# rogermm14/eonerf_code

Measured on AMD Instinct MI355X. Metric: train rays/sec on JAX_068 (4096 rays x 128 samples), higher is better.
Workload: dtype bf16

## Files before the change

eonerf_code_amd/csrc/eonerf_ctx.h:

```cpp
#pragma once
#include <hip/hip_runtime.h>
#include <string.h>
#include <algorithm>
#include <vector>
#include <unordered_map>

#include "../../include/eonerf_hip.h"
#include "eonerf_kernels.h"
#include "eonerf_pack.h"
#include "eonerf_rays.h"
#include "eonerf_carve.h"
#include "eonerf_wgrad_plan.h"

#define HIP_TRY(x) do { hipError_t e_ = (x); if (e_ != hipSuccess) return (int)e_; } while (0)

struct DevStream {
    uint8_t* data = nullptr; size_t bytes = 0;
    ChunkDesc* chunks = nullptr; int n_chunks = 0;
    PackEntry *e16 = nullptr, *e32 = nullptr, *e16lo = nullptr; int n16 = 0, n32 = 0, n16lo = 0;
};

constexpr int RANGE_WORD = 16;
constexpr int RANGE_STICKY_WORD = 17;
constexpr int DIGEST_WORD = 32;

struct eonerf_ctx {
    eonerf_config cfg;
    int n_samples = 128;
    int prec;
    bool bf16;
    int n_cu;
    int enc_pair = 1;
    int pipe_xcd = 0;
    int stagger = 0;
    int wgrad_riders = 1;
    ParamLayout pl;
    DevStream fwd_full, fwd_dens, bwd_full, bwd_dens, bwd_rgb, bwd_full_ig, pipe_wt, bwd_full_heads, bwd_rgb_heads, bwd_dens_heads, ig_tail_wt;
    bool pipe = false;
    int n_pipes = 0;
    float* loss_scratch = nullptr;
    float* fold = nullptr;
    bool pipe_fallback = true;
    bool need_repack = false;
    std::unordered_map<const void*, bool> ws_pipe;
    int pipe_fault_stage = -1;
    bool deterministic = false;
    unsigned long long* pipe_stamps = nullptr;
    uint64_t noise_seed = 0x5eed5eedULL; uint32_t noise_call = 0;
    struct Presample { bool valid = false; const void* ws = nullptr; const float* rays = nullptr; const int64_t* img_idx = nullptr;
                       const float* zsteps = nullptr; const int* count_out = nullptr; int n_rays = 0, flags = 0, n_samples = 0; bool pipe = false; uint32_t call = 0; } pre;
    hipEvent_t exch_event = nullptr; int exch_cus = 0; bool exch_recorded = false;
    const void* pre_consumed_ws = nullptr;
    bool full_ig_dirty = false;
    int* enc_colmap = nullptr;
    int* dev_status = nullptr;
    const uint32_t* occ_bits = nullptr; int occ_r = 0;
    bool weights_set = false;
    bool dens_dirty = false;
    bool dens_used = false;
    int prof_cap = 0;
    std::vector<hipEvent_t> prof_ev[EONERF_PROF_KERNELS][2];
    int prof_n[EONERF_PROF_KERNELS] = {};
};

inline CarveCfg carve_cfg(const eonerf_ctx* ctx) {
    CarveCfg c;
    c.bf16 = ctx->bf16; c.pipe = ctx->pipe; c.deterministic = ctx->deterministic; c.pipe_partials = ctx->deterministic;
    c.n_pipes = ctx->n_pipes; c.n_samples = ctx->n_samples;
    c.enc_part_wgs = (ctx->enc_pair && ctx->pipe && !ctx->deterministic) ? ctx->n_cu : 0;
    return c;
}
inline RenderWs carve_render(const eonerf_ctx* ctx, void* base, int n_rays, int flags) { return carve_render(carve_cfg(ctx), base, n_rays, flags); }

struct ProfScope {
    eonerf_ctx* c; int k; hipStream_t st; bool on;
    ProfScope(eonerf_ctx* ctx, int kernel, hipStream_t s) : c(ctx), k(kernel), st(s), on(kernel >= 0 && ctx->prof_cap > 0 && ctx->prof_n[kernel] < ctx->prof_cap) {
        if (on) (void)hipEventRecord(c->prof_ev[k][0][c->prof_n[k]], st);
    }
    ~ProfScope() { if (on) { (void)hipEventRecord(c->prof_ev[k][1][c->prof_n[k]], st); c->prof_n[k]++; } }
};

inline bool slabs_addressable(const eonerf_ctx* ctx, size_t p_cap) { return slab_blocks_addressable(ctx->bf16, p_cap); }
inline void drop_presample(eonerf_ctx* ctx, const void* ws) { if (ctx->pre.valid && ctx->pre.ws == ws) ctx->pre.valid = false; }
inline bool rays_in_range(const eonerf_ctx* ctx, int n_rays) { return n_rays <= (1 << 24) / (ctx->n_samples > 128 ? ctx->n_samples / 128 : 1); }
inline int chain_grid(const eonerf_ctx* ctx, int p_cap) { return std::min(ctx->n_cu, p_cap / (ctx->bf16 ? PBf16::TILE : PF32::TILE)); }

inline void note_train_forward(eonerf_ctx* ctx, const void* ws) {
    if (ctx->ws_pipe.size() > 1024) ctx->ws_pipe.clear();
    ctx->ws_pipe[ws] = ctx->pipe;
}
struct PipeModeGuard {
    eonerf_ctx* c; bool keep; const void* ws_; bool spend;
    PipeModeGuard(eonerf_ctx* ctx, const void* ws, bool spend_record = true) : c(ctx), keep(ctx->pipe), ws_(ws), spend(spend_record) {
        auto it = c->ws_pipe.find(ws);
        if (it != c->ws_pipe.end()) c->pipe = it->second;
    }
    ~PipeModeGuard() { c->pipe = keep; if (spend) c->ws_pipe.erase(ws_); }
};

inline AmbientW ambient_w(const eonerf_ctx* ctx, const float* flat) {
    const ParamLayout& pl = ctx->pl;
    return AmbientW{flat + pl.t[pl.am1_w].offset, flat + pl.t[pl.am1_b].offset, flat + pl.t[pl.am2_w].offset, flat + pl.t[pl.am2_b].offset};
}

inline int pipe_spare_cus(const eonerf_ctx* ctx) {
    const int spare = ctx->n_cu - ctx->n_pipes * PIPE_STAGES;
    return (ctx->pipe && !ctx->deterministic && spare >= 2) ? std::min(spare, 8) : 0;
}

inline MlpBwdArgs mlp_bwd_args(const eonerf_ctx* ctx, const PassBuffers& b, int p_cap, const DevStream& bs) {
    MlpBwdArgs m;
    memset(&m, 0, sizeof(m));
    m.stagger = ctx->stagger;
    m.n_pts = b.n_pts; m.p_pad = p_cap;
    m.stream = bs.data; m.chunks = bs.chunks; m.n_chunks = bs.n_chunks;
    m.sigma = b.sigma; m.albedo = b.albedo; m.ts = b.ts; m.tb = b.tb;
    m.g_sigma = b.g_sigma; m.g_albedo = b.g_albedo; m.g_ts = b.g_ts; m.g_tb = b.g_tb;
    m.masks = b.masks; m.grd = b.grd; m.g_emb = b.g_emb;
    m.px = b.px; m.py = b.py; m.pz = b.pz; m.g_pos = b.g_pos;
    return m;
}

int eo_pack(const eonerf_ctx* ctx, const std::vector<const DevStream*>& streams, const float* flat, hipStream_t st);
int eo_ensure_density_streams(eonerf_ctx* ctx, const float* flat, hipStream_t st);
int eo_sample_rays(eonerf_ctx* ctx, const float* rays, const float* zsteps, const float* u, int perturb, int n_rays, const uint32_t* bits, int r,
                   int64_t* ray_indices, float* t_starts, float* t_ends, float* pts_per_ray, int* n_dev, void* ws, size_t ws_bytes, void* stream);
int eo_run_mlp_fwd(eonerf_ctx* ctx, const PassBuffers& b, const float* flat, int p_cap, bool full, int mode, hipStream_t st, int prof_id = -1, bool render_train = false);
int eo_run_weight_gradients(eonerf_ctx* ctx, const float* flat, float* d_flat, const PassBuffers* full, const PassBuffers* dens, int p_cap, float* m_bott,
                            int* queue, hipStream_t st, WgradPlanOpts o, float* det_partials = nullptr, BottWgradArgs* defer_bott = nullptr);
```

eonerf_code_amd/csrc/eonerf_ctx.hip:

```cpp
#include <math.h>
#include <new>

#include "eonerf_ctx.h"

namespace {

int upload(DevStream& d, const PackedStream& s) {
    d.bytes = s.bytes; d.n_chunks = (int)s.chunks.size(); d.n16 = (int)s.e16.size(); d.n32 = (int)s.e32.size(); d.n16lo = (int)s.e16lo.size();
    HIP_TRY(hipMalloc(&d.data, s.bytes + 1024));
    HIP_TRY(hipMemset(d.data, 0, s.bytes + 1024));
    HIP_TRY(hipMalloc(&d.chunks, s.chunks.size() * sizeof(ChunkDesc)));
    HIP_TRY(hipMemcpy(d.chunks, s.chunks.data(), s.chunks.size() * sizeof(ChunkDesc), hipMemcpyHostToDevice));
    if (d.n16) {
        HIP_TRY(hipMalloc(&d.e16, s.e16.size() * sizeof(PackEntry)));
        HIP_TRY(hipMemcpy(d.e16, s.e16.data(), s.e16.size() * sizeof(PackEntry), hipMemcpyHostToDevice));
    }
    if (d.n32) {
        HIP_TRY(hipMalloc(&d.e32, s.e32.size() * sizeof(PackEntry)));
        HIP_TRY(hipMemcpy(d.e32, s.e32.data(), s.e32.size() * sizeof(PackEntry), hipMemcpyHostToDevice));
    }
    if (d.n16lo) {
        HIP_TRY(hipMalloc(&d.e16lo, s.e16lo.size() * sizeof(PackEntry)));
        HIP_TRY(hipMemcpy(d.e16lo, s.e16lo.data(), s.e16lo.size() * sizeof(PackEntry), hipMemcpyHostToDevice));
    }
// ... 47 lines not shown
    }
#pragma unroll
    for (int r = 0; r < 2; ++r) a.fold[(size_t)(o0 + r) * 256 + i] = (acc[r][0] + acc[r][1]) + (acc[r][2] + acc[r][3]);
#pragma unroll
    for (int r = 0; r < 2; ++r) a.wbt[(size_t)i * 256 + o0 + r] = a.w_b[(size_t)(o0 + r) * 256 + i];
    if (i < 2) {
        const int o = o0 + i;
        float b4[4] = {0.f, 0.f, 0.f, 0.f};
        for (int k = 0; k < 256; ++k) b4[k & 3] = fmaf(wat[i][k], a.b_b[k], b4[k & 3]);
        a.fold[256 * 256 + o] = ((b4[0] + b4[1]) + (b4[2] + b4[3])) + (o < 128 ? a.b_a1[o] : a.b_t1[o - 128]);
    }
}
constexpr float F16X3_W_MAX = 64.f, F16X3_W_MIN = 1.f / 512.f;
struct RangeJob { const float* w; int n; int check_min; };
struct RangeJobs { RangeJob j[24]; };
__global__ __launch_bounds__(256) void k_weight_range(RangeJobs jobs, int* range_flag) {
    __shared__ float red[256];
    __shared__ int bad[1];
    const RangeJob jb = jobs.j[blockIdx.x];
    if (threadIdx.x == 0) bad[0] = 0;
    __syncthreads();
    float m = 0.f;
    for (int i = threadIdx.x; i < jb.n; i += 256) {
        const float v = fabsf(jb.w[i]);
        if (!(v <= 3.0e38f)) bad[0] = 1;
        else m = fmaxf(m, v);
    }
    red[threadIdx.x] = m;
    __syncthreads();
    for (int o = 128; o > 0; o >>= 1) { if ((int)threadIdx.x < o) red[threadIdx.x] = fmaxf(red[threadIdx.x], red[threadIdx.x + o]); __syncthreads(); }
    if (threadIdx.x == 0) {
        const float mx = red[0];
        const float hi_lim = jb.check_min ? F16X3_W_MAX : 65504.f;
        if (bad[0] || mx > hi_lim || (jb.check_min && mx > 0.f && mx < F16X3_W_MIN)) atomicOr(range_flag + (RANGE_STICKY_WORD - RANGE_WORD), 1);
    }
}
int weight_range(const eonerf_ctx* ctx, const float* flat, hipStream_t st) {
    const ParamLayout& pl = ctx->pl;
    RangeJobs jobs;
    int n = 0;
    auto add = [&](int ti, int check_min) { jobs.j[n++] = RangeJob{flat + pl.t[ti].offset, pl.t[ti].rows * pl.t[ti].cols, check_min}; };
    for (int l = 0; l < 8; ++l) add(pl.trunk_w[l], 1);
    add(pl.sig_w, 1); add(pl.a2_w, 1);
    for (int l = 1; l < 4; ++l) add(pl.t_w[l], 1);
    add(pl.tsc_w, 1); add(pl.tbe_w, 1);
    add(pl.t_w[0], 0);
    add(pl.emb, 0);
    jobs.j[n++] = RangeJob{ctx->fold, 256 * 256, 1};
    hipLaunchKernelGGL(k_weight_range, dim3(n), dim3(256), 0, st, jobs, ctx->dev_status + RANGE_WORD);
    return (int)hipGetLastError();
}

int fold_heads(const eonerf_ctx* ctx, const float* flat, hipStream_t st) {
    const ParamLayout& pl = ctx->pl;
    FoldArgs a{flat + pl.t[pl.a1_w].offset, flat + pl.t[pl.a1_b].offset, flat + pl.t[pl.t_w[0]].offset, flat + pl.t[pl.t_b[0]].offset,
               flat + pl.t[pl.bot_w].offset, flat + pl.t[pl.bot_b].offset, ctx->fold, ctx->fold + FOLD_FLOATS};
    hipLaunchKernelGGL(k_fold, dim3(128), dim3(256), 0, st, a);
    return (int)hipGetLastError();
}

constexpr int CLOCK_PROBE_MFMAS = 8192;
typedef __attribute__((ext_vector_type(8))) __bf16 probe_bf16x8;
typedef __attribute__((ext_vector_type(16))) float probe_f32x16;
__global__ __launch_bounds__(256) void k_clock_probe(float* out) {
    probe_bf16x8 a, b;
#pragma unroll
    for (int e = 0; e < 8; ++e) { a[e] = (__bf16)(0.001f * (float)(threadIdx.x + e)); b[e] = (__bf16)(0.002f * (float)(threadIdx.x ^ e)); }
    probe_f32x16 c0 = {}, c1 = {}, c2 = {}, c3 = {};
    const unsigned long long t0 = __builtin_readcyclecounter(), r0 = __builtin_amdgcn_s_memrealtime();
    for (int i = 0; i < CLOCK_PROBE_MFMAS / 4; ++i) {
        c0 = __builtin_amdgcn_mfma_f32_32x32x16_bf16(a, b, c0, 0, 0, 0);
        c1 = __builtin_amdgcn_mfma_f32_32x32x16_bf16(a, b, c1, 0, 0, 0);
        c2 = __builtin_amdgcn_mfma_f32_32x32x16_bf16(a, b, c2, 0, 0, 0);
        c3 = __builtin_amdgcn_mfma_f32_32x32x16_bf16(a, b, c3, 0, 0, 0);
    }
    float s = 0.f;
#pragma unroll
    for (int e = 0; e < 16; ++e) s += (c0[e] + c1[e]) + (c2[e] + c3[e]);
    const unsigned long long t1 = __builtin_readcyclecounter(), r1 = __builtin_amdgcn_s_memrealtime();
    if (blockIdx.x == 0 && threadIdx.x == 0) {
        const float cyc = (float)(t1 - t0), ticks = (float)(r1 - r0);
        out[0] = cyc; out[1] = ticks; out[2] = ticks > 0.f ? cyc / ticks * 100.f : 0.f;
        out[3] = s == 12345.678f ? 1.f : 0.f;
    }
}

}

int eo_pack(const eonerf_ctx* ctx, const std::vector<const DevStream*>& streams, const float* flat, hipStream_t st) {
    PackJobs jobs;
    int n = 0, most = 1;
    auto flush = [&]() {
        if (n) hipLaunchKernelGGL(k_pack, dim3(std::min((most + 255) / 256, 1024), n), dim3(256), 0, st, flat, ctx->fold, (int)ctx->pl.total, jobs, ctx->dev_status + RANGE_WORD);
        n = 0; most = 1;
    };
    for (const DevStream* d : streams) {
        if (n + 3 > PACK_MAX_JOBS) flush();
        if (d->n16) jobs.j[n++] = PackJob{d->e16, d->n16, d->data, d->n16lo ? 2 : 1};
        if (d->n16lo) jobs.j[n++] = PackJob{d->e16lo, d->n16lo, d->data, 3};
        if (d->n32) jobs.j[n++] = PackJob{d->e32, d->n32, d->data, 0};
        most = std::max(most, std::max(d->n16, d->n32));
    }
    flush();
    return (int)hipGetLastError();
}

int eo_ensure_density_streams(eonerf_ctx* ctx, const float* flat, hipStream_t st) {
    ctx->dens_used = true;
    if (!ctx->dens_dirty) return 0;
    const int rc = ctx->prec == EONERF_F16X3 ? eo_pack(ctx, {&ctx->fwd_dens}, flat, st)
                 : ctx->pipe ? eo_pack(ctx, {&ctx->fwd_dens, &ctx->bwd_dens, &ctx->bwd_dens_heads, &ctx->ig_tail_wt}, flat, st)
                             : eo_pack(ctx, {&ctx->fwd_dens, &ctx->bwd_dens}, flat, st);
    if (!rc) ctx->dens_dirty = false;
    return rc;
}

extern "C" {

int eonerf_version(void) { return EONERF_VERSION; }

const char* eonerf_strerror(int code) {
    switch (code) {
        case EONERF_OK: return "ok";
        case EONERF_E_ARG: return "eonerf: invalid argument";
        case EONERF_E_WORKSPACE: return "eonerf: workspace too small";
        case EONERF_E_STATE: return "eonerf: call sequence error (set_weights / train forward missing, or a ray buffer refilled between eonerf_presample and its forward)";
        case EONERF_E_UNSUPPORTED: return "eonerf: unsupported configuration";
        case EONERF_E_RANGE: return "eonerf: a weight, an activation or a position left fp16's range (|v| > 65504 or not finite) in an fp16 x 3 call since the last check; its outputs are invalid -- render in fp32";
        case EONERF_E_DEVICE: return "eonerf: a device-side hand-off timed out (pipelined backward watchdog) on this or another rank; the gradients of that step are invalid and every optimizer update since has been skipped";
        default: return code > 0 ? hipGetErrorString((hipError_t)code) : "eonerf: unknown error";
    }
}

int eonerf_create(eonerf_ctx** out, const eonerf_config* cfg) {
    if (!out || !cfg || cfg->n_images < 1) return EONERF_E_ARG;
    if (cfg->n_samples < 2 || cfg->n_samples > 256) return EONERF_E_UNSUPPORTED;
    if (cfg->precision != EONERF_FP32 && cfg->precision != EONERF_BF16 && cfg->precision != EONERF_F16X3) return EONERF_E_ARG;
    eonerf_ctx* ctx = new (std::nothrow) eonerf_ctx();
    if (!ctx) return EONERF_E_ARG;
    ctx->cfg = *cfg;
    ctx->n_samples = cfg->n_samples;
    ctx->prec = cfg->precision;
    ctx->bf16 = cfg->precision == EONERF_BF16;
    const bool infer_only = cfg->precision == EONERF_F16X3;
    { const char* e = getenv("EONERF_DETERMINISTIC"); ctx->deterministic = e && atoi(e) != 0; }
    int dev = 0;
    hipDeviceProp_t prop;
    if (hipGetDevice(&dev) != hipSuccess || hipGetDeviceProperties(&prop, dev) != hipSuccess) { delete ctx; return (int)hipErrorNoDevice; }
    ctx->n_cu = prop.multiProcessorCount;
    { const char* e = getenv("EONERF_WGRAD_RIDERS"); if (e) ctx->wgrad_riders = atoi(e); }
    { const char* e = getenv("EONERF_STAGGER"); if (e) ctx->stagger = atoi(e); }
    { const char* e = getenv("EONERF_PIPE_XCD"); if (e) ctx->pipe_xcd = atoi(e); }
    { const char* e = getenv("EONERF_ENC_PAIR"); if (e) ctx->enc_pair = atoi(e); }
    ctx->pl.build(cfg->n_images);
    int rc = upload(ctx->fwd_full, build_fwd_stream(ctx->pl, ctx->prec, true));
    if (!rc) rc = upload(ctx->fwd_dens, build_fwd_stream(ctx->pl, ctx->prec, false));
    if (!rc && !infer_only) rc = upload(ctx->bwd_full, build_bwd_stream(ctx->pl, ctx->bf16, true, false));
    if (!rc && !infer_only) rc = upload(ctx->bwd_dens, build_bwd_stream(ctx->pl, ctx->bf16, false, true));
    if (!rc && !infer_only) rc = upload(ctx->bwd_rgb, build_bwd_stream(ctx->pl, ctx->bf16, true, false, false));
    if (!rc && !infer_only) rc = upload(ctx->bwd_full_ig, build_bwd_stream(ctx->pl, ctx->bf16, true, true, true));
    {
        const char* e = getenv("EONERF_PIPE");
        ctx->n_pipes = ctx->n_cu / PIPE_STAGES;
        ctx->pipe = ctx->bf16 && ctx->n_pipes >= 1 && !(e && atoi(e) == 0);
        if (ctx->pipe && !(e && atoi(e) == 1)) {
            if (!eo_bwd_pipe_fits_a_cu() || getenv("HSA_CU_MASK") || getenv("ROC_GLOBAL_CU_MASK")) ctx->pipe = false;
        }
        { const char* fb = getenv("EONERF_PIPE_FALLBACK"); ctx->pipe_fallback = !(fb && atoi(fb) == 0); }
        if (!rc && ctx->pipe) rc = upload(ctx->pipe_wt, build_pipe_stream(ctx->pl));
        if (!rc && ctx->pipe) rc = upload(ctx->bwd_full_heads, build_bwd_stream(ctx->pl, true, true, false, true, 1));
        if (!rc && ctx->pipe) rc = upload(ctx->bwd_rgb_heads, build_bwd_stream(ctx->pl, true, true, false, false, 1));
        if (!rc && ctx->pipe) rc = upload(ctx->bwd_dens_heads, build_bwd_stream(ctx->pl, true, false, true, false, 1));
        if (!rc && ctx->pipe) rc = upload(ctx->ig_tail_wt, build_ig_tail_stream(ctx->pl));
        { const char* f = getenv("EONERF_PIPE_FAULT"); ctx->pipe_fault_stage = f ? atoi(f) : -1; }
        { const char* f = getenv("EONERF_PIPE_STAMPS");
          if (!rc && ctx->pipe && f && atoi(f)) rc = (int)hipMalloc(&ctx->pipe_stamps, (size_t)ctx->n_pipes * PIPE_STAGES * 128 * sizeof(unsigned long long)); }
    }
    if (!rc) rc = (int)hipMalloc(&ctx->fold, (FOLD_FLOATS + 256 * 256) * sizeof(float));
    if (!rc) rc = (int)hipMalloc(&ctx->loss_scratch, (LOSS_MAX_BLOCKS + 4) * sizeof(float));
    if (!rc) rc = (int)hipMemset(ctx->loss_scratch, 0, (LOSS_MAX_BLOCKS + 4) * sizeof(float));
    if (!rc) rc = (int)hipMalloc(&ctx->dev_status, 64 * sizeof(int));
    if (!rc) rc = (int)hipMemset(ctx->dev_status, 0, 64 * sizeof(int));
    if (!rc) {
        int cm[64];
        for (int s = 0; s < 64; ++s) cm[s] = enc_col_of_slot(ctx->bf16, s);
        rc = (int)hipMalloc(&ctx->enc_colmap, sizeof(cm));
        if (!rc) rc = (int)hipMemcpy(ctx->enc_colmap, cm, sizeof(cm), hipMemcpyHostToDevice);
    }
    if (rc) { eonerf_destroy(ctx); return rc; }
    *out = ctx;
    return EONERF_OK;
}

int eonerf_profile_enable(eonerf_ctx* ctx, int max_launches) {
    if (!ctx || max_launches < 0) return EONERF_E_ARG;
    for (int k = 0; k < EONERF_PROF_KERNELS; ++k) {
        for (int s = 0; s < 2; ++s) {
            for (hipEvent_t e : ctx->prof_ev[k][s]) (void)hipEventDestroy(e);
            ctx->prof_ev[k][s].clear();
            for (int i = 0; i < max_launches; ++i) { hipEvent_t e; HIP_TRY(hipEventCreate(&e)); ctx->prof_ev[k][s].push_back(e); }
        }
        ctx->prof_n[k] = 0;
    }
    ctx->prof_cap = max_launches;
    return EONERF_OK;
}

int eonerf_clock_probe(eonerf_ctx* ctx, float* out4, void* stream) {
    if (!ctx || !out4) return EONERF_E_ARG;
    hipLaunchKernelGGL(k_clock_probe, dim3(ctx->n_cu), dim3(256), 0, (hipStream_t)stream, out4);
    return (int)hipGetLastError();
}

const char* eonerf_profile_name(int kernel) {
    static const char* const names[EONERF_PROF_KERNELS] = {"fwd_chain_camera", "bwd_chain_camera", "wgrad_gemm", "fwd_chain_sun", "bwd_chain_sun",
                                                           "bwd_pipe_camera", "bwd_pipe_sun", "ig_tail_sun"};
    return kernel >= 0 && kernel < EONERF_PROF_KERNELS ? names[kernel] : nullptr;
}

int eonerf_profile_read(eonerf_ctx* ctx, int kernel, float* total_ms, int* launches) {
    if (!ctx || kernel < 0 || kernel >= EONERF_PROF_KERNELS || !total_ms || !launches) return EONERF_E_ARG;
    float sum = 0.f;
    for (int i = 0; i < ctx->prof_n[kernel]; ++i) {
        HIP_TRY(hipEventSynchronize(ctx->prof_ev[kernel][1][i]));
        float ms = 0.f;
        HIP_TRY(hipEventElapsedTime(&ms, ctx->prof_ev[kernel][0][i], ctx->prof_ev[kernel][1][i]));
        sum += ms;
    }
    *total_ms = sum; *launches = ctx->prof_n[kernel];
    return EONERF_OK;
}

int eonerf_destroy(eonerf_ctx* ctx) {
    if (!ctx) return EONERF_E_ARG;
    for (int k = 0; k < EONERF_PROF_KERNELS; ++k) for (int s = 0; s < 2; ++s) for (hipEvent_t e : ctx->prof_ev[k][s]) (void)hipEventDestroy(e);
    release(ctx->fwd_full); release(ctx->fwd_dens); release(ctx->bwd_full); release(ctx->bwd_dens); release(ctx->bwd_rgb); release(ctx->bwd_full_ig); release(ctx->pipe_wt); release(ctx->bwd_full_heads); release(ctx->bwd_rgb_heads); release(ctx->bwd_dens_heads); release(ctx->ig_tail_wt);
    if (ctx->fold) (void)hipFree(ctx->fold);
    if (ctx->loss_scratch) (void)hipFree(ctx->loss_scratch);
    if (ctx->enc_colmap) (void)hipFree(ctx->enc_colmap);
    if (ctx->pipe_stamps) (void)hipFree(ctx->pipe_stamps);
    if (ctx->dev_status) (void)hipFree(ctx->dev_status);
    delete ctx;
    return EONERF_OK;
}

int eonerf_param_tensors(const eonerf_ctx* ctx) { return ctx ? (int)ctx->pl.t.size() : 0; }
size_t eonerf_param_floats(const eonerf_ctx* ctx) { return ctx ? ctx->pl.total : 0; }
int eonerf_param_info(const eonerf_ctx* ctx, int index, const char** name, size_t* offset, int* rows, int* cols) {
    if (!ctx || index < 0 || index >= (int)ctx->pl.t.size()) return EONERF_E_ARG;
    const ParamInfo& p = ctx->pl.t[index];
    if (name) *name = p.name.c_str();
    if (offset) *offset = p.offset;
    if (rows) *rows = p.rows;
    if (cols) *cols = p.cols;
    return EONERF_OK;
}

int eonerf_set_weights(eonerf_ctx* ctx, const float* flat, void* stream) {
    if (!ctx || !flat) return EONERF_E_ARG;
    hipStream_t st = (hipStream_t)stream;
    std::vector<const DevStream*> v;
    v.push_back(&ctx->fwd_full);
    if (ctx->prec == EONERF_F16X3) {}
    else if (ctx->pipe) { v.push_back(&ctx->bwd_full_heads); v.push_back(&ctx->bwd_rgb_heads); }
    else { v.push_back(&ctx->bwd_full); v.push_back(&ctx->bwd_rgb); }
    if (ctx->pipe) v.push_back(&ctx->pipe_wt);
    const bool with_dens = ctx->dens_used;
    if (with_dens) {
        v.push_back(&ctx->fwd_dens);
        if (ctx->prec != EONERF_F16X3) v.push_back(&ctx->bwd_dens);
        if (ctx->pipe) { v.push_back(&ctx->bwd_dens_heads); v.push_back(&ctx->ig_tail_wt); }
    }
    ctx->need_repack = false;
    int rc = fold_heads(ctx, flat, st);
    if (!rc && ctx->prec == EONERF_F16X3) {
        rc = (int)hipMemsetAsync(ctx->dev_status + RANGE_STICKY_WORD, 0, sizeof(int), st);
        if (!rc) rc = weight_range(ctx, flat, st);
    }
    if (!rc) rc = eo_pack(ctx, v, flat, st);
    if (!rc) { ctx->weights_set = true; ctx->dens_dirty = !with_dens; ctx->full_ig_dirty = true; ctx->dens_used = false; }
    return rc;
}

int eonerf_debug_pipe_stamps(eonerf_ctx* ctx, unsigned long long* host_out, int capacity) {
    if (!ctx || !ctx->pipe_stamps || !host_out) return 0;
    const int n = ctx->n_pipes * PIPE_STAGES * 128;
    if (capacity < n) return 0;
    if (hipDeviceSynchronize() != hipSuccess) return 0;
    if (hipMemcpy(host_out, ctx->pipe_stamps, (size_t)n * sizeof(unsigned long long), hipMemcpyDeviceToHost) != hipSuccess) return 0;
    return n;
}

int eonerf_device_status(eonerf_ctx* ctx, void* stream) {
    if (!ctx) return EONERF_E_ARG;
    int err = 0;
    HIP_TRY(hipMemcpyAsync(&err, ctx->dev_status, sizeof(int), hipMemcpyDeviceToHost, (hipStream_t)stream));
    HIP_TRY(hipStreamSynchronize((hipStream_t)stream));
    if (!err) return EONERF_OK;
    HIP_TRY(hipMemsetAsync(ctx->dev_status, 0, sizeof(int), (hipStream_t)stream));
    if ((err & ~0x100) == EO_STATUS_PRESAMPLE_STALE) return EONERF_E_STATE;
    if (ctx->pipe && ctx->pipe_fallback) { ctx->pipe = false; ctx->need_repack = true; }
    return EONERF_E_DEVICE;
}

int eonerf_range_status(eonerf_ctx* ctx, void* stream) {
    if (!ctx) return EONERF_E_ARG;
// ... 53 lines not shown
```

eonerf_code_amd/csrc/eonerf_kernels.h:

```cpp
#pragma once
#include <hip/hip_runtime.h>
#include <stdint.h>
#include "eonerf_common.h"
#include "eonerf_rays.h"

struct EoAttrOnce {
    bool done[64] = {};
    template <class F> hipError_t ensure(F&& set) {
        int dev = -1;
        if (hipGetDevice(&dev) != hipSuccess || dev < 0 || dev >= 64) return set();
        if (done[dev]) return hipSuccess;
        const hipError_t e = set();
        if (e == hipSuccess) done[dev] = true;
        return e;
    }
};

constexpr int ACT_ROW_ENC = 0;
constexpr int ACT_ROW_X1 = 64;
constexpr int ACT_ROW_HEADS = 64 + 8 * 256;
constexpr int ACT_ROW_A1 = ACT_ROW_HEADS;
constexpr int ACT_ROW_T1 = ACT_ROW_A1 + 128;
constexpr int ACT_ROW_EMB = ACT_ROW_T1 + 512;
constexpr int ACT_ROWS_FULL = ACT_ROW_EMB + 32;
constexpr int ACT_ROWS_DENSITY = ACT_ROW_HEADS;

constexpr int GRD_ROW_Y0 = 0;
constexpr int GRD_ROW_SIG = 8 * 256;
constexpr int GRD_ROW_A2 = GRD_ROW_SIG + 32;
constexpr int GRD_ROW_A1 = GRD_ROW_A2 + 32;
constexpr int GRD_ROW_T1 = GRD_ROW_A1 + 128;
constexpr int GRD_ROW_T5 = GRD_ROW_T1 + 512;
constexpr int GRD_ROWS_FULL = GRD_ROW_T5 + 32;
constexpr int GRD_ROWS_DENSITY = GRD_ROW_SIG + 32;

struct ActMap {
    __host__ __device__ static constexpr SlabBlk block(int row) {
        if (row < ACT_ROW_X1) return SlabBlk{ACT_ROW_ENC, 64};
        if (row < ACT_ROW_A1) return SlabBlk{ACT_ROW_X1 + (row - ACT_ROW_X1) / 256 * 256, 256};
        if (row < ACT_ROW_EMB) return SlabBlk{ACT_ROW_A1 + (row - ACT_ROW_A1) / 128 * 128, 128};
        return SlabBlk{ACT_ROW_EMB, 32};
    }
};
struct GrdMap {
    __host__ __device__ static constexpr SlabBlk block(int row) {
        if (row < GRD_ROW_SIG) return SlabBlk{row / 256 * 256, 256};
        if (row < GRD_ROW_A2) return SlabBlk{GRD_ROW_SIG, 32};
        if (row < GRD_ROW_A1) return SlabBlk{GRD_ROW_A2, 32};
        if (row < GRD_ROW_T1 + 128) return SlabBlk{GRD_ROW_A1, 256};
        if (row < GRD_ROW_T5) return SlabBlk{GRD_ROW_T1 + (row - GRD_ROW_T1) / 128 * 128, 128};
        return SlabBlk{GRD_ROW_T5, 32};
    }
};

constexpr int MASK_SLOTS_FULL = 13;
constexpr int MASK_SLOTS_DENSITY = 8;

template <class P> struct FwdSlot { static constexpr int BYTES = chunk_target<P>() * P::UNIT_B + 1024; };

struct MlpFwdArgs {
    const float *px, *py, *pz;
    const int* simg;
    const float* emb;
    const int* n_pts;
    int p_pad;
    const uint8_t* stream;
    const ChunkDesc* chunks;
    int n_chunks;
    float *sigma, *albedo, *ts, *tb;
    void* act;
    uint32_t* masks;
    int mask_from;
    int* range_flag;
    int stagger;
};

struct MlpBwdArgs {
    const int* n_pts;
    int p_pad;
    const uint8_t* stream;
    const ChunkDesc* chunks;
    int n_chunks;
    const float *sigma, *albedo, *ts, *tb;
    const float *g_sigma, *g_albedo, *g_ts, *g_tb;
    const uint32_t* masks;
    void* grd;
    float* g_emb;
    const float *px, *py, *pz;
    float* g_pos;
    uint8_t* dy7_units;
    int stagger;
};

struct WgradJob {
    const void* a;
    const void* b;
    uint32_t a_stride, b_stride;
    float* dw;
    float* db;
    float* dw2;
    float* db2;
    int split, dw2_ld;
    const int* col_map;
    const int* n_pts;
    int m_rows, n_rows;
    int dw_ld;
    int gm, gn, wm, wn;
    int item0, slices;
    int a_units;
};

constexpr int PIPE_STAGES = 7;
constexpr int PIPE_MAX_STAGES = 7;
constexpr int PIPE_TS = 32;
constexpr int PIPE_RING = 16;
constexpr int PIPE_UNIT_B = 16 * 1024;
struct BwdPipeArgs {
    const int* n_pts; int p_pad;
    int n_pipes;
    int n_stages;
    const uint8_t* wt;
    const uint8_t* dy_in;
    const void* act;
    void* grd;
    uint8_t* rings;
    uint32_t* flags;
    uint32_t* scratch_word;
    int* role_counter;
    int xcd_local;
    int* error;
    float* d_flat;
    size_t dw_off[PIPE_MAX_STAGES], db_off[PIPE_MAX_STAGES];
    int dw_ld[PIPE_MAX_STAGES];
    unsigned long long* stamps;
    float* partials;
    int fault_stage;
    int amb_blocks;
    AmbientBwdArgs amb;
};
hipError_t eo_launch_bwd_pipe(const BwdPipeArgs& a, hipStream_t st);
struct IgTailArgs {
    const int* n_pts; int p_pad;
    const void* grd;
    const uint8_t* wt;
    const float *px, *py, *pz;
    float* g_pos;
};
hipError_t eo_launch_ig_tail(const IgTailArgs& a, int n_wg, hipStream_t st);
struct EncPairArgs {
    const int* n_pts; int p_pad;
    const void* grd;
    const void* act;
    const uint8_t* wt;
    const float *px, *py, *pz;
    float* g_pos;
    float* part;
};
hipError_t eo_launch_enc_pair(const EncPairArgs& a, int n_wg, hipStream_t st);
size_t eo_bwd_pipe_lds_bytes();
bool eo_bwd_pipe_fits_a_cu();

hipError_t eo_launch_mlp_fwd(const MlpFwdArgs& a, int prec, bool full, int mode, int grid, hipStream_t st);
hipError_t eo_launch_mlp_bwd(const MlpBwdArgs& a, bool bf16, bool full, bool input_grad, bool transient, int grid, hipStream_t st, int pipe = 0);
constexpr int WGRAD_MAX_JOBS = 32;
static_assert(sizeof(WgradJob) * WGRAD_MAX_JOBS + 8 + 64 <= 4096, "job table exceeds the kernel-argument segment");
struct WgradAux {
    int job;
    int emb_row0, emb_ld;
    uint32_t a2_stride, b2_stride;
    const void* a2;
    const void* b2;
    float *dw_sig, *db_sig, *dw_emb;
};
struct WgradJobTable { WgradJob j[WGRAD_MAX_JOBS]; WgradAux aux; int n; int items; };
constexpr int WGRAD_PART_F = 256 * 256 + 256;
hipError_t eo_launch_wgrad(const WgradJobTable& jobs, int n_wg, int p_pad, int* queue, bool bf16, hipStream_t st, float* partials = nullptr,
                           bool zero_queue = true);
hipError_t eo_launch_pipe_reduce(const BwdPipeArgs& a, hipStream_t st);
```

eonerf_code_amd/csrc/eonerf_render.hip:

```cpp
#include "eonerf_ctx.h"
#include "eonerf_render_args.h"

int eo_run_mlp_fwd(eonerf_ctx* ctx, const PassBuffers& b, const float* flat, int p_cap, bool full, int mode, hipStream_t st, int prof_id, bool render_train) {
    if (!full) { const int rc = eo_ensure_density_streams(ctx, flat, st); if (rc) return rc; }
    const DevStream& ds = full ? ctx->fwd_full : ctx->fwd_dens;
    MlpFwdArgs a;
    a.px = b.px; a.py = b.py; a.pz = b.pz; a.simg = b.simg;
    a.emb = flat + ctx->pl.t[ctx->pl.emb].offset;
    a.n_pts = b.n_pts; a.p_pad = p_cap;
    a.stream = ds.data; a.chunks = ds.chunks; a.n_chunks = ds.n_chunks;
    a.sigma = b.sigma; a.albedo = b.albedo; a.ts = b.ts; a.tb = b.tb;
    a.act = b.act; a.masks = b.masks;
    a.range_flag = ctx->dev_status + RANGE_WORD;
    a.stagger = ctx->stagger;
    a.mask_from = (render_train && ctx->pipe) ? 7 : 0;
    if (ctx->prec == EONERF_F16X3 && mode != 0) return EONERF_E_UNSUPPORTED;
    ProfScope ps(ctx, prof_id, st);
    return (int)eo_launch_mlp_fwd(a, ctx->prec, full, mode, chain_grid(ctx, p_cap), st);
}

static int run_bwd_pipe(eonerf_ctx* ctx, const RenderWs& w, const PassBuffers& b, int p_cap, float* d_flat, int prof_id, hipStream_t st, int slot, bool first_of_backward,
                        const AmbientBwdArgs* amb = nullptr) {
    const ParamLayout& pl = ctx->pl;
    if (first_of_backward) { const ZeroSpan z = backward_zero_span(w); HIP_TRY(hipMemsetAsync(z.base, 0, z.bytes, st)); }
// ... 228 lines not shown
    PipeModeGuard mode(ctx, ws);
    const int flags = EONERF_F_TRAIN | (depth_only ? EONERF_F_ONLY_DEPTH : 0);
    RenderWs w = carve_render(ctx, ws, n_rays, flags);
    if (ctx->pre.valid && ctx->pre.ws == ws) return EONERF_E_STATE;
    if (ws_bytes < w.bytes) return EONERF_E_WORKSPACE;
    const int p_cap = p_cap_of(n_rays, ctx->n_samples);
    RenderingOutBwdArgs rb{w.ray_rec, n_rays, depth_only ? nullptr : g_albedo, g_depth, depth_only ? nullptr : g_beta,
                           depth_only ? nullptr : g_transient_s, depth_only ? nullptr : g_ambient, w.g_ray};
    HIP_TRY(eo_launch_rendering_out_bwd(rb, st));
    return camera_backward(ctx, w, flat, rays, img_idx, n_rays, p_cap, d_flat, true, !depth_only, true, nullptr, depth_only != 0, st);
}

int eonerf_presample(eonerf_ctx* ctx, const float* rays, const int64_t* img_idx, const float* zsteps, int n_rays, int flags,
                     int* n_samples_dev, void* ws, size_t ws_bytes, void* stream) {
    hipStream_t st = (hipStream_t)stream;
    if (!ctx || !rays || !img_idx || !zsteps || n_rays < 0 || !ws) return EONERF_E_ARG;
    if (!(flags & EONERF_F_TRAIN) || (flags & EONERF_F_ONLY_DEPTH)) return EONERF_E_STATE;
    ctx->pre.valid = false;
    if (n_rays == 0) return EONERF_OK;
    if (!rays_in_range(ctx, n_rays) || !slabs_addressable(ctx, (size_t)p_cap_of(n_rays, ctx->n_samples))) return EONERF_E_UNSUPPORTED;
    RenderWs w = carve_render(ctx, ws, n_rays, flags);
    if (ws_bytes < w.bytes) return EONERF_E_WORKSPACE;
    SampleArgs sa = camera_sample_args(ctx, w, rays, img_idx, zsteps, nullptr, nullptr, n_rays, n_samples_dev);
    sa.call = ctx->noise_call++;
    unsigned long long* digest = reinterpret_cast<unsigned long long*>(ctx->dev_status + DIGEST_WORD);
    HIP_TRY(hipMemsetAsync(digest, 0, 2 * sizeof(unsigned long long), st));
    sa.digest = digest;
    HIP_TRY(eo_launch_sampler(sa, st));
    eonerf_ctx::Presample& p = ctx->pre;
    p.valid = true; p.ws = ws; p.rays = rays; p.img_idx = img_idx; p.zsteps = zsteps; p.count_out = n_samples_dev; p.n_rays = n_rays; p.flags = flags;
    p.n_samples = ctx->n_samples; p.pipe = ctx->pipe; p.call = sa.call;
    return EONERF_OK;
}

int eonerf_presample_cancel(eonerf_ctx* ctx) {
    if (!ctx) return EONERF_E_ARG;
    ctx->pre.valid = false;
    return EONERF_OK;
}

int eonerf_render_forward(eonerf_ctx* ctx, const float* flat, const float* rays, const int64_t* img_idx,
                          const float* zsteps, const float* u_cam, const float* u_retry, const float* u_sun,
                          int n_rays, int flags, float* out, int* n_samples_dev,
                          void* ws, size_t ws_bytes, void* stream) {
    hipStream_t st = (hipStream_t)stream;
    if (!ctx || !flat || !rays || !img_idx || !zsteps || !out || n_rays < 0 || !ws) return EONERF_E_ARG;
    if (!ctx->weights_set) return EONERF_E_STATE;
    if (n_rays == 0) return EONERF_OK;
    if (ctx->need_repack) { const int rcr = eonerf_set_weights(ctx, flat, stream); if (rcr) return rcr; }
    const bool shadows = (flags & EONERF_F_SHADOWS) && !(flags & EONERF_F_ONLY_DEPTH);
    const bool train = flags & EONERF_F_TRAIN, od = flags & EONERF_F_ONLY_DEPTH;
    const bool philox = u_cam == nullptr;
    if (philox ? (u_retry || u_sun) : (shadows && !u_sun)) return EONERF_E_ARG;
    if (train && od) return EONERF_E_UNSUPPORTED;
    if (!rays_in_range(ctx, n_rays) || (train && !slabs_addressable(ctx, (size_t)p_cap_of(n_rays, ctx->n_samples)))) return EONERF_E_UNSUPPORTED;
    RenderWs w = carve_render(ctx, ws, n_rays, flags);
    if (ws_bytes < w.bytes) return EONERF_E_WORKSPACE;
    if (train) note_train_forward(ctx, ws);
    const int p_cap = p_cap_of(n_rays, ctx->n_samples);

    const eonerf_ctx::Presample pre = ctx->pre;
    const bool presampled = pre.valid && philox && pre.ws == ws && pre.rays == rays && pre.img_idx == img_idx && pre.zsteps == zsteps &&
                            pre.count_out == n_samples_dev && pre.n_rays == n_rays && pre.flags == flags && pre.n_samples == ctx->n_samples && pre.pipe == ctx->pipe;
    ctx->pre.valid = false;
    ctx->pre_consumed_ws = (presampled && train) ? ws : nullptr;
    SampleArgs sa = camera_sample_args(ctx, w, rays, img_idx, zsteps, u_cam, u_retry, n_rays, n_samples_dev, !train);
    if (presampled) sa.call = pre.call;
    else {
        if (philox) sa.call = ctx->noise_call++;
        HIP_TRY(eo_launch_sampler(sa, st));
    }
    const bool rgb_loss = train && !shadows && (flags & EONERF_F_RGB_LOSS);
    int rc = eo_run_mlp_fwd(ctx, w.cam, flat, p_cap, !od, train ? (rgb_loss ? 2 : 1) : 0, st, EONERF_PROF_FWD_CHAIN_CAMERA, train);
    if (rc) return rc;
    const ShadeArgs sh = shade_args(ctx, w, flat, img_idx, n_rays, shadows, flags, out);
    const SampleArgs ss = sun_sample_args(sa, w, u_sun);
    const CompositeArgs ca = camera_composite_args(ctx, w, flat, rays, n_rays, p_cap, od, sh, shadows, ss);
    HIP_TRY(eo_launch_composite_fwd(ca, st));

    if (shadows) {
        HIP_TRY(eo_launch_sampler(ss, st, true));
        rc = eo_run_mlp_fwd(ctx, w.sun, flat, p_cap, false, train ? 1 : 0, st, EONERF_PROF_FWD_CHAIN_SUN, train);
        if (rc) return rc;
        HIP_TRY(eo_launch_composite_fwd(shadow_composite_args(ca, w), st));
    }
    return EONERF_OK;
}

static bool render_backward_refused(eonerf_ctx* ctx, const float* flat, const float* rays, const int64_t* img_idx, int n_rays, int flags,
                                    const float* d_flat, const void* ws, size_t ws_bytes, bool spend, int* rc) {
    auto with = [&](int code) { *rc = code; return true; };
    if (!ctx || !flat || !rays || !img_idx || !d_flat || n_rays < 0 || !ws) return with(EONERF_E_ARG);
    if (!(flags & EONERF_F_TRAIN) || (flags & EONERF_F_ONLY_DEPTH)) return with(EONERF_E_STATE);
    if (ctx->prec == EONERF_F16X3) return with(EONERF_E_UNSUPPORTED);
    if (!ctx->weights_set) return with(EONERF_E_STATE);
    if (n_rays == 0) return with(EONERF_OK);
    if (!rays_in_range(ctx, n_rays) || !slabs_addressable(ctx, (size_t)p_cap_of(n_rays, ctx->n_samples))) return with(EONERF_E_UNSUPPORTED);
    PipeModeGuard mode(ctx, ws, false);
    const int bad = (ctx->pre.valid && ctx->pre.ws == ws) ? EONERF_E_STATE
                  : ws_bytes < carve_render(ctx, nullptr, n_rays, flags).bytes ? EONERF_E_WORKSPACE : EONERF_OK;
    if (bad && spend) ctx->ws_pipe.erase(ws);
    return bad ? with(bad) : false;
}

struct LossSpec { const float *out, *pixels; int kind; float* loss; };
static int render_backward_impl(eonerf_ctx* ctx, const float* flat, const float* rays, const int64_t* img_idx,
                                int n_rays, int flags, const float* d_out, const LossSpec* ls, float* d_flat,
                                void* ws, size_t ws_bytes, void* stream) {
    hipStream_t st = (hipStream_t)stream;
    int refusal;
    if (render_backward_refused(ctx, flat, rays, img_idx, n_rays, flags, d_flat, ws, ws_bytes, true, &refusal)) return refusal;
    PipeModeGuard mode(ctx, ws);
    const bool shadows = flags & EONERF_F_SHADOWS;
    ctx->exch_recorded = false;
    RenderWs w = carve_render(ctx, ws, n_rays, flags);
    const int p_cap = p_cap_of(n_rays, ctx->n_samples);
    const ParamLayout& pl = ctx->pl;
    const int grid = chain_grid(ctx, p_cap);
    auto dptr = [&](int ti) { return d_flat + pl.t[ti].offset; };

    ShadeBwdArgs sb;
    sb.ray_rec = w.ray_rec; sb.d_out = d_out; sb.img_idx = img_idx;
    sb.loss_kind = -1; sb.loss_out = nullptr; sb.loss_gt = nullptr; sb.loss = nullptr; sb.loss_scratch = nullptr;
    if (ls) { sb.loss_kind = ls->kind; sb.loss_out = ls->out; sb.loss_gt = ls->pixels; sb.loss = ls->loss; sb.loss_scratch = ctx->loss_scratch; }
    sb.radiometric = ctx->cfg.radiometric ? flat + pl.t[pl.rad].offset : nullptr;
    sb.d_radiometric = ctx->cfg.radiometric ? dptr(pl.rad) : nullptr;
    sb.g_ray = w.g_ray; sb.n_rays = n_rays; sb.use_shadow = shadows ? 1 : 0; sb.eval = (flags & EONERF_F_EVAL) ? 1 : 0;
    sb.lds_images = ctx->cfg.n_images <= 2048 ? ctx->cfg.n_images : 0;
    sb.d_rad_rays = sb.d_radiometric ? w.det.rad_rays : nullptr;
    const bool chk = ctx->pre_consumed_ws == ws;
    ctx->pre_consumed_ws = nullptr;
    unsigned long long* digest = reinterpret_cast<unsigned long long*>(ctx->dev_status + DIGEST_WORD);
    sb.chk_rays = chk ? rays : nullptr; sb.chk_sum = chk ? digest + 1 : nullptr;
    const bool prezeroed = ctx->pipe && w.pipe.dy_in;
    sb.zero_base = nullptr; sb.zero_bytes = 0;
    if (prezeroed) {
        const ZeroSpan z = backward_zero_span(w);
        sb.zero_base = reinterpret_cast<uint32_t*>(z.base); sb.zero_bytes = z.bytes;
        if ((reinterpret_cast<uintptr_t>(z.base) | z.bytes) & 15) return EONERF_E_STATE;
    }
    HIP_TRY(eo_launch_shade_bwd(sb, st));
    if (sb.d_rad_rays) HIP_TRY(eo_launch_table_reduce(sb.d_rad_rays, img_idx, n_rays, 6, 9, ctx->cfg.n_images, sb.eval, sb.d_radiometric, st));

    CompositeBwdArgs cb;
    memset(&cb, 0, sizeof(cb));
    cb.n_samples = ctx->n_samples;
    cb.rays = rays; cb.p_pad = p_cap; cb.n_rays = n_rays; cb.ray_rec = w.ray_rec; cb.g_ray = w.g_ray;
    bool ambient_done = false, sun_enc_done = false;

    if (shadows) {
        CompositeBwdArgs cs = cb;
        cs.offsets = w.sun.offsets; cs.counts = w.sun.counts; cs.sigma = w.sun.sigma; cs.delta = w.sun.delta;
        cs.g_sigma = w.sun.g_sigma; cs.g_pos = w.sun.g_pos;
        HIP_TRY(eo_launch_sun_composite_bwd(cs, st));
        const bool pipe_sun = ctx->pipe && w.pipe.dy_in;
        MlpBwdArgs ms = mlp_bwd_args(ctx, w.sun, p_cap, pipe_sun ? ctx->bwd_dens_heads : ctx->bwd_dens);
        if (pipe_sun) {
            ms.dy7_units = w.pipe.dy_in;
            { ProfScope ps(ctx, EONERF_PROF_BWD_CHAIN_SUN, st); HIP_TRY(eo_launch_mlp_bwd(ms, true, false, true, false, grid, st, true)); }
            const AmbientBwdArgs ag = ambient_bwd_args(ctx, w, flat, rays, n_rays, d_flat);
            ambient_done = pipe_spare_cus(ctx) > 0;
            const int rcp = run_bwd_pipe(ctx, w, w.sun, p_cap, d_flat, EONERF_PROF_BWD_PIPE_SUN, st, 0, !prezeroed, ambient_done ? &ag : nullptr);
            if (rcp) return rcp;
            if (w.enc_part) {
                EncPairArgs ea;
                ea.n_pts = w.sun.n_pts; ea.p_pad = p_cap; ea.grd = w.sun.grd; ea.act = w.sun.act; ea.wt = ctx->ig_tail_wt.data;
                ea.px = w.sun.px; ea.py = w.sun.py; ea.pz = w.sun.pz; ea.g_pos = w.sun.g_pos;
                ea.part = w.enc_part;
                { ProfScope ps(ctx, EONERF_PROF_IG_TAIL_SUN, st); HIP_TRY(eo_launch_enc_pair(ea, ctx->n_cu, st)); }
                sun_enc_done = true;
            } else {
                IgTailArgs ta;
                ta.n_pts = w.sun.n_pts; ta.p_pad = p_cap; ta.grd = w.sun.grd; ta.wt = ctx->ig_tail_wt.data;
                ta.px = w.sun.px; ta.py = w.sun.py; ta.pz = w.sun.pz; ta.g_pos = w.sun.g_pos;
                { ProfScope ps(ctx, EONERF_PROF_IG_TAIL_SUN, st); HIP_TRY(eo_launch_ig_tail(ta, ctx->n_cu, st)); }
            }
        } else {
            ProfScope ps(ctx, EONERF_PROF_BWD_CHAIN_SUN, st);
            HIP_TRY(eo_launch_mlp_bwd(ms, ctx->bf16, false, true, false, grid, st));
        }
    }

    const int rcc = camera_backward(ctx, w, flat, rays, img_idx, n_rays, p_cap, d_flat, shadows || !(flags & EONERF_F_RGB_LOSS), shadows && !ambient_done, !shadows && !prezeroed,
                                    shadows ? &w.sun : nullptr, false, st, chk ? digest : nullptr, sun_enc_done);
    if (!rcc && ctx->exch_event && !ctx->exch_recorded) HIP_TRY(hipEventRecord(ctx->exch_event, st));
    return rcc;
}

int eonerf_render_backward(eonerf_ctx* ctx, const float* flat, const float* rays, const int64_t* img_idx,
                           int n_rays, int flags, const float* d_out, float* d_flat,
                           void* ws, size_t ws_bytes, void* stream) {
    if (!d_out) return EONERF_E_ARG;
    return render_backward_impl(ctx, flat, rays, img_idx, n_rays, flags, d_out, nullptr, d_flat, ws, ws_bytes, stream);
}

int eonerf_render_backward_loss(eonerf_ctx* ctx, const float* flat, const float* rays, const int64_t* img_idx,
                                int n_rays, int flags, const float* out, const float* pixels, int kind, float* d_out_scratch, float* loss,
                                float* d_flat, void* ws, size_t ws_bytes, void* stream) {
    if (!ctx || !out || !pixels || !loss || (kind != 0 && kind != 1) || n_rays < 1) return EONERF_E_ARG;
    if ((n_rays + 255) / 256 > LOSS_MAX_BLOCKS) {
        if (!d_out_scratch) return EONERF_E_ARG;
        int rc;
        if (render_backward_refused(ctx, flat, rays, img_idx, n_rays, flags, d_flat, ws, ws_bytes, false, &rc)) return rc;
        rc = eonerf_train_loss(ctx, out, pixels, n_rays, kind, d_out_scratch, loss, stream);
        return rc ? rc : render_backward_impl(ctx, flat, rays, img_idx, n_rays, flags, d_out_scratch, nullptr, d_flat, ws, ws_bytes, stream);
    }
    const LossSpec ls{out, pixels, kind, loss};
    return render_backward_impl(ctx, flat, rays, img_idx, n_rays, flags, nullptr, &ls, d_flat, ws, ws_bytes, stream);
}

}
```

Baseline: 1.264 million.

## Fuse sun composite backward and sigma-head MLP backward into one kernel

```diff
diff --git a/eonerf_code_amd/csrc/eonerf_ctx.h b/eonerf_code_amd/csrc/eonerf_ctx.h
--- a/eonerf_code_amd/csrc/eonerf_ctx.h
+++ b/eonerf_code_amd/csrc/eonerf_ctx.h
@@ -31,6 +31,7 @@
     bool bf16;
     int n_cu;
     int enc_pair = 1;
+    int fused_seams = 1;
     int pipe_xcd = 0;
     int stagger = 0;
     int wgrad_riders = 1;
diff --git a/eonerf_code_amd/csrc/eonerf_ctx.hip b/eonerf_code_amd/csrc/eonerf_ctx.hip
--- a/eonerf_code_amd/csrc/eonerf_ctx.hip
+++ b/eonerf_code_amd/csrc/eonerf_ctx.hip
@@ -223,6 +223,7 @@
     { const char* e = getenv("EONERF_STAGGER"); if (e) ctx->stagger = atoi(e); }
     { const char* e = getenv("EONERF_PIPE_XCD"); if (e) ctx->pipe_xcd = atoi(e); }
     { const char* e = getenv("EONERF_ENC_PAIR"); if (e) ctx->enc_pair = atoi(e); }
+    { const char* e = getenv("EONERF_FUSED_SEAMS"); if (e) ctx->fused_seams = atoi(e); }
     ctx->pl.build(cfg->n_images);
     int rc = upload(ctx->fwd_full, build_fwd_stream(ctx->pl, ctx->prec, true));
     if (!rc) rc = upload(ctx->fwd_dens, build_fwd_stream(ctx->pl, ctx->prec, false));
diff --git a/eonerf_code_amd/csrc/eonerf_kernels.h b/eonerf_code_amd/csrc/eonerf_kernels.h
--- a/eonerf_code_amd/csrc/eonerf_kernels.h
+++ b/eonerf_code_amd/csrc/eonerf_kernels.h
@@ -162,6 +162,17 @@
 
 hipError_t eo_launch_mlp_fwd(const MlpFwdArgs& a, int prec, bool full, int mode, int grid, hipStream_t st);
 hipError_t eo_launch_mlp_bwd(const MlpBwdArgs& a, bool bf16, bool full, bool input_grad, bool transient, int grid, hipStream_t st, int pipe = 0);
+struct SunSigmaBwdArgs {
+    const int* n_pts; int p_pad;
+    const int *offsets, *counts; int n_rays;
+    const float *ray_rec, *g_ray;
+    const float *sigma, *delta;
+    const uint32_t* masks;
+    const uint8_t* w_units;
+    void* grd;
+    uint8_t* dy7_units;
+};
+hipError_t eo_launch_sun_sigma_bwd(const SunSigmaBwdArgs& a, hipStream_t st);
 constexpr int WGRAD_MAX_JOBS = 32;
 static_assert(sizeof(WgradJob) * WGRAD_MAX_JOBS + 8 + 64 <= 4096, "job table exceeds the kernel-argument segment");
 struct WgradAux {
diff --git a/eonerf_code_amd/csrc/eonerf_render.hip b/eonerf_code_amd/csrc/eonerf_render.hip
--- a/eonerf_code_amd/csrc/eonerf_render.hip
+++ b/eonerf_code_amd/csrc/eonerf_render.hip
@@ -404,12 +404,20 @@
         CompositeBwdArgs cs = cb;
         cs.offsets = w.sun.offsets; cs.counts = w.sun.counts; cs.sigma = w.sun.sigma; cs.delta = w.sun.delta;
         cs.g_sigma = w.sun.g_sigma; cs.g_pos = w.sun.g_pos;
-        HIP_TRY(eo_launch_sun_composite_bwd(cs, st));
         const bool pipe_sun = ctx->pipe && w.pipe.dy_in;
+        const bool one_kernel = pipe_sun && ctx->fused_seams;
+        if (!one_kernel) HIP_TRY(eo_launch_sun_composite_bwd(cs, st));
         MlpBwdArgs ms = mlp_bwd_args(ctx, w.sun, p_cap, pipe_sun ? ctx->bwd_dens_heads : ctx->bwd_dens);
         if (pipe_sun) {
             ms.dy7_units = w.pipe.dy_in;
-            { ProfScope ps(ctx, EONERF_PROF_BWD_CHAIN_SUN, st); HIP_TRY(eo_launch_mlp_bwd(ms, true, false, true, false, grid, st, true)); }
+            if (one_kernel) {
+                SunSigmaBwdArgs sg;
+                sg.n_pts = w.sun.n_pts; sg.p_pad = p_cap; sg.offsets = cs.offsets; sg.counts = cs.counts; sg.n_rays = n_rays;
+                sg.ray_rec = w.ray_rec; sg.g_ray = w.g_ray; sg.sigma = w.sun.sigma; sg.delta = w.sun.delta; sg.masks = w.sun.masks;
+                sg.w_units = ctx->bwd_dens_heads.data; sg.grd = w.sun.grd; sg.dy7_units = w.pipe.dy_in;
+                ProfScope ps(ctx, EONERF_PROF_BWD_CHAIN_SUN, st);
+                HIP_TRY(eo_launch_sun_sigma_bwd(sg, st));
+            } else { ProfScope ps(ctx, EONERF_PROF_BWD_CHAIN_SUN, st); HIP_TRY(eo_launch_mlp_bwd(ms, true, false, true, false, grid, st, true)); }
             const AmbientBwdArgs ag = ambient_bwd_args(ctx, w, flat, rays, n_rays, d_flat);
             ambient_done = pipe_spare_cus(ctx) > 0;
             const int rcp = run_bwd_pipe(ctx, w, w.sun, p_cap, d_flat, EONERF_PROF_BWD_PIPE_SUN, st, 0, !prezeroed, ambient_done ? &ag : nullptr);
diff --git a/eonerf_code_amd/csrc/eonerf_sun_sigma_bwd.hip b/eonerf_code_amd/csrc/eonerf_sun_sigma_bwd.hip
--- /dev/null
+++ b/eonerf_code_amd/csrc/eonerf_sun_sigma_bwd.hip
@@ -0,0 +1,88 @@
+#include "eonerf_common.h"
+#include "eonerf_kernels.h"
+
+namespace {
+
+constexpr int SSB_WAVES = 4;
+
+__global__ __launch_bounds__(64 * SSB_WAVES) void k_sun_sigma_bwd(SunSigmaBwdArgs a) {
+    __shared__ __attribute__((aligned(16))) uint16_t s_w[2 * 16 * 8];
+    const int tid = threadIdx.x, lane = tid & 63, wave = __builtin_amdgcn_readfirstlane(tid >> 6), h = lane >> 5, c = lane & 31;
+    const int n_pts = *a.n_pts;
+    const int n_wt = (n_pts + PBf16::TILE - 1) / PBf16::TILE * PBf16::WAVES;
+    if ((int)blockIdx.x * SSB_WAVES >= n_wt) return;
+    {
+        const int f = tid;
+        const int kg = f >> 4, rem = f & 15;
+        s_w[((rem >> 2) & 1) * 128 + kg * 8 + (rem >> 3) * 4 + (rem & 3)] =
+            *reinterpret_cast<const uint16_t*>(a.w_units + (size_t)(f >> 5) * PBf16::UNIT_B + (f & 31) * 16);
+    }
+    __syncthreads();
+    const int wt = (int)blockIdx.x * SSB_WAVES + wave;
+    if (wt >= n_wt) return;
+    const int p0 = wt * 32, p = p0 + c;
+    const bool live = p < n_pts;
+    const u32x4 mk = *reinterpret_cast<const u32x4*>(a.masks + ((size_t)7 * a.p_pad * 2 + (size_t)p * 2 + h) * 4);
+    const float sg = a.sigma[p], dl = a.delta[p];
+
+    float dsig = 0.f;
+    if (p0 < n_pts) {
+        int lo = 0, span = a.n_rays, v;
+        for (;;) {
+            const int step = (span + 63) >> 6, idx = lo + lane * step;
+            v = idx < (step == 1 ? a.n_rays : lo + span) ? a.offsets[idx] : 0x7fffffff;
+            if (step == 1) break;
+            const int k = __popcll(__builtin_amdgcn_ballot_w64(v <= p0)) - 1, end = lo + span;
+            lo += k * step;
+            span = end - lo < step ? end - lo : step;
+        }
+        const int j0 = __popcll(__builtin_amdgcn_ballot_w64(v <= p0)) - 1, j1 = __popcll(__builtin_amdgcn_ballot_w64(v <= p0 + 31)) - 1;
+        int ray = lo + j0;
+        for (int j = j0 + 1; j <= j1; ++j) ray += __builtin_amdgcn_readlane(v, j) <= p ? 1 : 0;
+        if (j1 == 63 && lo + 64 < a.n_rays) {
+            int hi = a.n_rays;
+            while (hi - ray > 1) {
+                const int mid = (ray + hi) >> 1;
+                if (a.offsets[mid] <= p) ray = mid; else hi = mid;
+            }
+        }
+        if (live) {
+            const int i = p - a.offsets[ray], n = a.counts[ray];
+            const float g_geo = a.g_ray[(size_t)ray * RAY_REC + RR_GEO], geo = a.ray_rec[(size_t)ray * RAY_REC + RR_GEO];
+            const float g_sigma = i < n - 1 ? -g_geo * geo * dl : 0.f;
+            dsig = g_sigma * (1.f - expf(-sg));
+        }
+    }
+    SlabWriter<PBf16, GrdMap> sw;
+    sw.init(a.grd, a.p_pad / Slab<PBf16>::TSAMP, wt * 32, lane, nullptr);
+    sw.elem(GRD_ROW_SIG, h == 0 ? dsig : 0.f);
+
+    const float d = (float)(__bf16)dsig;
+    uint8_t* dst = a.dy7_units + (size_t)wt * PIPE_UNIT_B + lane * 16;
+#pragma unroll
+    for (int kg = 0; kg < 16; ++kg) {
+        const u32x4 wv = *reinterpret_cast<const u32x4*>(s_w + h * 128 + kg * 8);
+        const int mt = kg >> 1;
+        const uint32_t m = mk[mt >> 1];
+        u32x4 o;
+#pragma unroll
+        for (int w = 0; w < 4; ++w) {
+            const int s = 4 * (kg & 1) + w, pos = 8 * (mt & 1) + 7 - s;
+            const uint32_t sel = (m >> pos) & 0x00010001u;
+            const float w0 = __uint_as_float(wv[w] << 16), w1 = __uint_as_float(wv[w] & 0xffff0000u);
+            const uint32_t wi = cvt_pk_bf16(__builtin_fmaf(w0, d, 0.f), __builtin_fmaf(w1, d, 0.f));
+            uint32_t r;
+            asm("v_pk_mul_lo_u16 %0, %1, %2" : "=v"(r) : "v"(wi), "v"(sel));
+            o[w] = r;
+        }
+        *reinterpret_cast<u32x4*>(dst + kg * 1024) = o;
+    }
+}
+
+}
+
+hipError_t eo_launch_sun_sigma_bwd(const SunSigmaBwdArgs& a, hipStream_t st) {
+    if (!a.dy7_units || !a.w_units || a.n_rays < 1 || a.p_pad % PBf16::TILE) return hipErrorInvalidValue;
+    hipLaunchKernelGGL(k_sun_sigma_bwd, dim3(a.p_pad / (32 * SSB_WAVES)), dim3(64 * SSB_WAVES), 0, st, a);
+    return hipGetLastError();
+}
```

After: 1.268 million (median of 6 runs). Within noise of the previous version (+0.3%).
